# rflamino/monte_carlo_retirement

Hardware: AMD Instinct MI355X
Metric: paths/sec (whole node), config.json scenario, 833-month paths, success-count only (higher is better)
Workload: dtype f64

## Files before the change

### monte_carlo_retirement_amd/csrc/mcr_hip.hip

```cpp

#include <hip/hip_runtime.h>

#include <climits>
#include <cmath>
#include <cstdarg>
#include <cstdio>
#include <cstdlib>
#include <cstring>
#include <algorithm>
#include <mutex>
#include <thread>
#include <type_traits>
#include <utility>
#include <vector>

#include "mcr_device.h"
#include "mcr_numpy_rng.h"
#include "mcr_screen.h"
#include "mcr_host.h"

namespace mcr {

constexpr int kMaxSegments = 8;
constexpr int kRngHistorySchemes = 3;
// ... 1001 lines not shown
    if (kSliced && seg >= 0 && seg < io.seg_q - 1) {
        const bool hand_over = seg == 0 || __hip_atomic_load(&seg_ok_s, __ATOMIC_RELAXED, __HIP_MEMORY_SCOPE_WORKGROUP) != 0;
        if (hand_over) {
            *seg_at(0) = b1; *seg_at(1) = b2; *seg_at(2) = c1; *seg_at(3) = c2;
            if (ANNUAL) { *seg_at(4) = gacc1; *seg_at(5) = gacc2; }
            *seg_at(6) = infl;
            store_bits(seg_at(7), (alive ? 1ull : 0ull) | (succeeded ? 2ull : 0ull) | ((unsigned long long)(ruin_bin + 1) << 8) | ((unsigned long long)done_years << 24));
            store_bits(seg_at(8), ((unsigned long long)carry.w3 << 32) | (unsigned long long)carry.w2);
            for (int k = 0; k < P.n_lock_slots; ++k) *seg_at(kSegFixedFields + k) = lock_lds[(size_t)k * kBlock + tid];
            if (MODE >= 1) {
                *seg_at(9) = start_balance; *seg_at(10) = infl_ret;
                *seg_at(11) = sum_col[0]; *seg_at(12) = sum_col[kBlock]; *seg_at(13) = sum_col[2 * kBlock];
            }
            __builtin_amdgcn_fence(__ATOMIC_RELEASE, "agent");
        }
        __syncthreads();
        if (threadIdx.x == 0)
            __hip_atomic_store(io.seg_flags + (size_t)seg_block * (size_t)io.seg_q + (size_t)seg, hand_over ? 1u : 2u, __ATOMIC_RELEASE, __HIP_MEMORY_SCOPE_AGENT);
        return;
    }

    if (P.total_months % kMPY != 0) {
        if (succeeded) {
            const bool tf = annual_gain_taxes<false, TANY, ANNUAL, T1, T2, MM, TOL, EQR>(P, L, b1, c1, b2, c2, gacc1, gacc2);
            if (tf) {
                succeeded = false; ruin_bin = ry + 1;
                if (kSumLds) sum_col[2 * kBlock] = (double)ry; else ytr_bits = f64_bits((double)ry);
                if constexpr (OUT) RM.month = kMPY * ry;
            }
            if constexpr (kBins) YB.last = b1 + b2;
            else put_sample(P.trajectory_len - 1, b1 + b2, infl);
        }
        if constexpr (kBins) year_bins_row(io.yb, YB.L, YB.k++, valid, P.trajectory_len - 1, true, YB.last, infl, -1, kNanBits);
    }
    const double final_balance = fmax(0.0, b1 + b2);

    if (kSumLds) { fy_gross = sum_col[0]; fy_real = sum_col[kBlock]; ytr_bits = f64_bits(sum_col[2 * kBlock]); }
    if (kSummary && valid) {
        const mcr_outputs& o = io.out;
        if (o.start_balance) o.start_balance[li] = start_balance;
        if (o.final_balance) o.final_balance[li] = final_balance;
        if (o.years_to_ruin) store_bits(&o.years_to_ruin[li], ytr_bits);
        if (o.first_year_gross_withdrawal) o.first_year_gross_withdrawal[li] = fy_gross;
        if (o.first_year_real_gross_withdrawal) o.first_year_real_gross_withdrawal[li] = fy_real;
        if (o.inflation_at_retirement) o.inflation_at_retirement[li] = infl_ret;
        if (o.success) o.success[li] = succeeded ? 1 : 0;
    }
#ifdef MCR_K1_TIMELINE
    if (MODE == 0 && RNG == 0 && io.path_seeds && (threadIdx.x & 63) == 0) {
        unsigned long long* tl = (unsigned long long*)io.path_seeds + ((size_t)blockIdx.x * 4 + (threadIdx.x >> 6)) * 3;
        tl[0] = tl_t0; tl[1] = wall_clock64();
        tl[2] = ((unsigned long long)__builtin_amdgcn_s_getreg(20 | (31 << 11)) << 32) | __builtin_amdgcn_s_getreg(4 | (31 << 11));
    }
#endif
    const unsigned long long ok = __builtin_amdgcn_ballot_w64(valid && succeeded);
    if (kFan) {
        if ((threadIdx.x & 63) == 0) blk[fan_j] = (unsigned int)__popcll(ok);
        if constexpr (kScnFan) {
            const int fan_n = late_arg<int32_t>(offsetof(KernelIO, fan_n));
            const uint64_t n_paths = late_arg<uint64_t>(offsetof(KernelIO, n_paths));
            uint64_t* const fan_ctr = late_arg<uint64_t*>(offsetof(KernelIO, out) + offsetof(mcr_outputs, counters));
            uint64_t* const fan_masks = late_arg<uint64_t*>(offsetof(KernelIO, fan_masks));
            if (fan_masks && (threadIdx.x & 63) == 0) fan_masks[(size_t)fan_j * ((n_paths + 63) >> 6) + path_block] = ok;
            if constexpr (OUT) {
                double* const fan_final = late_arg<double*>(offsetof(KernelIO, fan_rows) + offsetof(KernelIO::FanRows, final_balance));
                double* const fan_ruin = late_arg<double*>(offsetof(KernelIO, fan_rows) + offsetof(KernelIO::FanRows, years_to_ruin));
                const int64_t row_stride = late_arg<int64_t>(offsetof(KernelIO, fan_rows) + offsetof(KernelIO::FanRows, row_stride));
                const uint64_t col = (uint64_t)path_block * kPaths + (threadIdx.x & 63);
                if (col < n_paths) {
                    const size_t at = (size_t)fan_j * (size_t)row_stride + (size_t)col;
                    if (fan_final) store_bits(&fan_final[at], succeeded ? f64_bits(final_balance) : kNanBits);
                    if (fan_ruin) store_bits(&fan_ruin[at], RM.month < 0 ? kNanBits : f64_bits((double)RM.month / (double)kMPY));
                }
            }
            __syncthreads();
            if (threadIdx.x < (unsigned)fan_n && fan_ctr) {
                uint64_t* c = fan_ctr + (size_t)threadIdx.x * MCR_N_COUNTERS;
                const uint64_t first = (uint64_t)path_block * kPaths;
                const uint64_t cnt = n_paths - first < (uint64_t)kPaths ? n_paths - first : (uint64_t)kPaths;
                atomicAdd((unsigned long long*)&c[MCR_CTR_SUCCESS], (unsigned long long)blk[threadIdx.x]);
                atomicAdd((unsigned long long*)&c[MCR_CTR_PATHS], (unsigned long long)cnt);
            }
            return;
        }
        __syncthreads();
        uint64_t* const fan_ctr = kGrid ? cell->counters : io.out.counters;
        if (threadIdx.x < (unsigned)io.fan_n && fan_ctr) {
            uint64_t* c = fan_ctr + (size_t)threadIdx.x * MCR_N_COUNTERS;
            const uint64_t first = (uint64_t)path_block * kPaths;
            const uint64_t cnt = io.n_paths - first < (uint64_t)kPaths ? io.n_paths - first : (uint64_t)kPaths;
            atomicAdd((unsigned long long*)&c[MCR_CTR_SUCCESS], (unsigned long long)blk[threadIdx.x]);
            atomicAdd((unsigned long long*)&c[MCR_CTR_PATHS], (unsigned long long)cnt);
        }
        return;
    }
    if ((threadIdx.x & 63) == 0) atomicAdd(&blk[0], (unsigned int)__popcll(ok));
    const bool want_bins = io.out.ruin_year_bins != nullptr || io.out.wr_obs_counts != nullptr;
    if (want_bins && valid) {
        if (ruin_bin >= 0) atomicAdd(&blk[1 + ruin_bin], 1u);
        atomicAdd(&blk[1 + (ry + 2) + done_years], 1u);
    }
    if ((PHASE == 0 || PHASE == 3) && n_hist > 0 && valid && succeeded) {
        const double* __restrict__ e = io.out.hist_edges;
        if (final_balance >= e[0] && final_balance <= e[n_hist]) {
            int lo = 0, hi = n_hist;
            while (hi - lo > 1) {
                const int mid = (lo + hi) >> 1;
                if (e[mid] <= final_balance) lo = mid; else hi = mid;
            }
            atomicAdd(&blk[n_blk + lo], 1u);
        }
    }
    if constexpr (kBins) { if (io.yb.final_success && valid && succeeded) atomicAdd(&YB.L.fin[year_bins_cell(YB.L.edges, YB.L.n, final_balance)], 1u); }
    __syncthreads();
    if constexpr (kBins) year_bins_flush_final(io.yb, YB.L);
    uint64_t* ctr = io.out.counters ? io.out.counters + (kCand ? (size_t)io.cand_out[cand] * MCR_N_COUNTERS : 0) : nullptr;
    if (threadIdx.x == 0 && ctr) {
        atomicAdd((unsigned long long*)&ctr[MCR_CTR_SUCCESS], (unsigned long long)blk[0]);
        const uint64_t first = (uint64_t)path_block * kPaths;
        const uint64_t cnt = io.n_paths - first < (uint64_t)kPaths ? io.n_paths - first : (uint64_t)kPaths;
        if constexpr (LIST) {
            const uint64_t list_n = *io.path_list_count;
            atomicAdd((unsigned long long*)&ctr[MCR_CTR_PATHS], (unsigned long long)(list_n - first < (uint64_t)kPaths ? list_n - first : (uint64_t)kPaths));
        } else
        atomicAdd((unsigned long long*)&ctr[MCR_CTR_PATHS], (unsigned long long)cnt);
    }
    if (want_bins) {
        for (int k = threadIdx.x; k < ry + 2; k += kPaths) {
            if (io.out.ruin_year_bins && blk[1 + k])
                atomicAdd((unsigned long long*)&io.out.ruin_year_bins[k], (unsigned long long)blk[1 + k]);
        }
        for (int y = threadIdx.x; y < ry; y += kPaths) {
            unsigned int c = 0;
            for (int d = y + 1; d <= ry; ++d) c += blk[1 + (ry + 2) + d];
            if (io.out.wr_obs_counts && c)
                atomicAdd((unsigned long long*)&io.out.wr_obs_counts[y], (unsigned long long)c);
        }
    }
    for (int k = threadIdx.x; k < n_hist; k += kPaths)
        if (blk[n_blk + k]) atomicAdd((unsigned long long*)&io.out.hist_bins[k], (unsigned long long)blk[n_blk + k]);
}

struct ScreenIO {
    uint64_t seed, path_begin, n_paths;
    uint32_t stream_id, reserved;
    uint64_t* counters;
    uint64_t* wr_obs_counts;
    uint32_t* list;
    uint32_t* list_count;
    uint8_t* cls;
    float* min_ratio;
    float* final_total;
};
template <int TAXED, bool EQR, bool HOOK = false>
__global__ __launch_bounds__(kBlock, 8) void screen_kernel(const ScreenParams S, const ScreenIO io) {
    static_assert(TAXED >= 0 && TAXED <= 3 && (!EQR || TAXED == 3), "TAXED is path_kernel's mask; equal rates need both assets taxed");
    constexpr bool T1 = (TAXED & 1) != 0, T2 = (TAXED & 2) != 0;
    __shared__ unsigned int safe_s;
    if (threadIdx.x == 0) safe_s = 0u;
    __syncthreads();
    const uint64_t local = (uint64_t)blockIdx.x * kBlock + threadIdx.x;
    const bool valid = local < io.n_paths;
    const uint64_t path = io.path_begin + (valid ? local : io.n_paths - 1);
    const PhiloxPath PQ = philox_path(path, io.stream_id, io.seed);
    float b1 = S.b1_0, b2 = S.b2_0, c1 = b1, c2 = b2, infl = 1.0f;
    float peak = b1 + b2;
    float contrib = S.contrib, k1 = contrib * S.alloc1, k2 = contrib - k1;
    bool ok = __builtin_fminf(b1, b2) > kScreenMinBalance;
    [[maybe_unused]] float min_ratio = __builtin_inff();
    PairCarry carry{0u, 0u};
    const int wm = S.working_months, total = S.total_months;
    int moy = 0;
    const int prio_t1 = (total / 2) & ~1, prio_t2 = ((total * 3) / 4) & ~1, prio_t3 = ((total * 9) / 10) & ~1;
    int prio_next = prio_t1;
    __builtin_amdgcn_s_setprio(3);
    for (int row = 0; row < total; row += 2) {
        if (__builtin_amdgcn_ballot_w64(ok) == 0ull) break;
        if (row == prio_next) {
            if (row == prio_t1) __builtin_amdgcn_s_setprio(2);
            else if (row == prio_t2) __builtin_amdgcn_s_setprio(1);
            else if (row == prio_t3) __builtin_amdgcn_s_setprio(0);
            prio_next = prio_from(prio_t1, prio_t2, prio_t3, row + 2);
        }
        float g[6];
        if (PQ.hi_uniform) {
            if ((row & 2) == 0) screen_factors2<0, true>(S, PQ, io.seed, (uint32_t)row >> 2, carry, g);
            else screen_factors2<1, true>(S, PQ, io.seed, (uint32_t)row >> 2, carry, g);
        } else {
            if ((row & 2) == 0) screen_factors2<0, false>(S, PQ, io.seed, (uint32_t)row >> 2, carry, g);
            else screen_factors2<1, false>(S, PQ, io.seed, (uint32_t)row >> 2, carry, g);
        }
#pragma unroll
        for (int r = 0; r < 2; ++r) {
            const int m = row + r;
            if (m >= total) break;
            const float g1 = g[3 * r], ginf = g[3 * r + 1], g2 = g[3 * r + 2];
            if (m < wm) {
                if (moy == kMPY) {
                    moy = 0;
                    if (S.contrib_grows) { contrib *= S.contrib_growth_factor; k1 = contrib * S.alloc1; k2 = contrib - k1; }
                }
                ++moy;
                b1 *= g1; b2 *= g2; infl *= ginf;
                b1 += k1; c1 += k1; b2 += k2; c2 += k2;
            } else {
                const float price = infl;
                float income = S.expenses * price;
                if ((unsigned)(m - S.s0) < S.n0) income = __builtin_fmaf(-S.sa0, price, income);
                if ((unsigned)(m - S.s1) < S.n1) income = __builtin_fmaf(-S.sa1, price, income);
                const float need = __builtin_fmaxf(0.0f, income);
                b1 *= g1; b2 *= g2; infl *= ginf;
                const float v1 = T1 ? __builtin_fmaf(-__builtin_fmaxf(0.0f, b1 - c1), S.rate1, b1) : b1;
                const float v2 = T2 ? __builtin_fmaf(-__builtin_fmaxf(0.0f, b2 - c2), EQR ? S.rate1 : S.rate2, b2) : b2;
                const float cap = v1 + v2;
                ok = ok && cap >= kScreenNeedMargin * need && cap >= peak * (1.0f / kScreenPeakDiv);
                const float inv_cap = __builtin_amdgcn_rcpf(cap);
                const float phi = __builtin_fminf(need, cap) * inv_cap;
                if constexpr (HOOK) { if (need > 0.0f) min_ratio = __builtin_fminf(min_ratio, cap * __builtin_amdgcn_rcpf(need)); }
                b1 = __builtin_fmaf(-b1, phi, b1); c1 = __builtin_fmaf(-c1, phi, c1);
                b2 = __builtin_fmaf(-b2, phi, b2); c2 = __builtin_fmaf(-c2, phi, c2);
            }
            peak = __builtin_fmaxf(peak, screen_rebalance<TAXED, EQR>(S, b1, c1, b2, c2));
            ok = ok && __builtin_fminf(b1, b2) > kScreenMinBalance;
        }
    }
    ok = ok && peak < kScreenMaxTotal;
    const bool safe = valid && ok, doubt = valid && !ok;
    const unsigned long long safe_mask = __builtin_amdgcn_ballot_w64(safe), doubt_mask = __builtin_amdgcn_ballot_w64(doubt);
    const unsigned int lane = threadIdx.x & 63u;
    if (lane == 0u && safe_mask) atomicAdd(&safe_s, (unsigned int)__popcll(safe_mask));
    if (io.list && doubt_mask) {
        unsigned int base = 0u;
        if (lane == 0u) base = atomicAdd(io.list_count, (unsigned int)__popcll(doubt_mask));
        base = (unsigned int)__builtin_amdgcn_readfirstlane((int)base);
        const unsigned int before = __builtin_amdgcn_mbcnt_hi((unsigned int)(doubt_mask >> 32), __builtin_amdgcn_mbcnt_lo((unsigned int)doubt_mask, 0u));
        if (doubt) io.list[base + before] = (uint32_t)local;
    }
    if constexpr (HOOK) {
        if (valid) {
            if (io.cls) io.cls[local] = ok ? MCR_SCREEN_SAFE : MCR_SCREEN_DOUBTFUL;
            if (io.min_ratio) io.min_ratio[local] = min_ratio;
            if (io.final_total) io.final_total[local] = b1 + b2;
        }
    }
    __syncthreads();
    const unsigned int n_safe = safe_s;
    if (n_safe == 0u) return;
    if (threadIdx.x == 0 && io.counters) {
        atomicAdd((unsigned long long*)&io.counters[MCR_CTR_SUCCESS], (unsigned long long)n_safe);
        atomicAdd((unsigned long long*)&io.counters[MCR_CTR_PATHS], (unsigned long long)n_safe);
    }
    if (io.wr_obs_counts)
        for (int y = threadIdx.x; y < S.retirement_years; y += kBlock) atomicAdd((unsigned long long*)&io.wr_obs_counts[y], (unsigned long long)n_safe);
}

__global__ void exp_forms_kernel(const double* in, double* out, int64_t n) {
    __shared__ double tab[kTabDoubles], tab_c[kTabDoubles];
    load_math_tables(tab, threadIdx.x, blockDim.x);
    load_math_tables<true>(tab_c, threadIdx.x, blockDim.x);
    __syncthreads();
    const int64_t i = (int64_t)blockIdx.x * blockDim.x + threadIdx.x;
    if (i >= n) return;
    out[2 * i] = fexp<true>(in[i], tab, MathRegs::literals_path());
    out[2 * i + 1] = fexp<true, true>(in[i], tab_c, MathRegs::literals_path());
}
__global__ void helper_kernel(int which, const DevParams P, const double* in, double* out, int64_t n) {
    __shared__ double tab[kTabDoubles];
    load_math_tables(tab, threadIdx.x, blockDim.x);
    __syncthreads();
    const int64_t i = (int64_t)blockIdx.x * blockDim.x + threadIdx.x;
    if (i >= n) return;
    switch (which) {
        case MCR_HELPER_WITHDRAW: {
            const double* x = in + 5 * i;
            double bal = x[0], cb = x[1], g, nt;
            const double rate = (x[3] != 0.0 && x[4] > 0.0) ? x[4] : 0.0;
            withdraw(bal, cb, x[2], rate, g, nt);
            out[4 * i + 0] = bal; out[4 * i + 1] = cb; out[4 * i + 2] = g; out[4 * i + 3] = nt;
            break;
        }
        case MCR_HELPER_NLV: {
            const double* x = in + 4 * i;
            const double rate = (x[2] != 0.0 && x[3] > 0.0) ? x[3] : 0.0;
            out[i] = net_liquidation_value(x[0], x[1], rate);
            break;
        }
        case MCR_HELPER_REBALANCE: {
            const double* x = in + 4 * i;
            double b1 = x[0], c1 = x[1], b2 = x[2], c2 = x[3];
            rebalance(lane_params(P), b1, c1, b2, c2);
            out[4 * i + 0] = b1; out[4 * i + 1] = c1; out[4 * i + 2] = b2; out[4 * i + 3] = c2;
            break;
        }
        case MCR_HELPER_ANNUAL_TAX: {
            const double* x = in + 6 * i;
            double b1 = x[0], c1 = x[1], b2 = x[2], c2 = x[3];
            const bool tf = annual_gain_taxes(P, lane_params(P), b1, c1, b2, c2, x[4], x[5]);
            out[5 * i + 0] = b1; out[5 * i + 1] = c1; out[5 * i + 2] = b2; out[5 * i + 3] = c2;
            out[5 * i + 4] = tf ? 1.0 : 0.0;
            break;
        }
        case MCR_HELPER_MONTHLY_GROSS: {
            const double* x = in + 3 * i;
            out[i] = monthly_gross(x[0] / (double)kMPY, x[1] / sqrt((double)kMPY), x[2], tab);
            break;
        }
        case MCR_HELPER_MATH_EXP: out[i] = fexp(in[i], tab, MathRegs::literals()); break;
        case MCR_HELPER_MATH_DIV: out[i] = fdiv(in[2 * i], in[2 * i + 1]); break;
        case MCR_HELPER_MATH_DIV_PATH: out[i] = fdiv<false>(in[2 * i], in[2 * i + 1]); break;
        case MCR_HELPER_MATH_SQRT: out[i] = fsqrt(in[i]); break;
        case MCR_HELPER_WITHDRAW2_PATH: {
            const double* x = in + 6 * i;
            const LaneParams L = lane_params(P);
            double b1 = x[0], c1 = x[1], b2 = x[3], c2 = x[4], g1, n1, g2, n2;
            switch (P.tax_mask) {
                case 0: withdraw2<false, false>(b1, c1, x[2], L.real_rate1, g1, n1, b2, c2, x[5], L.real_rate2, g2, n2); break;
                case 1: withdraw2<true, false>(b1, c1, x[2], L.real_rate1, g1, n1, b2, c2, x[5], L.real_rate2, g2, n2); break;
                case 2: withdraw2<false, true>(b1, c1, x[2], L.real_rate1, g1, n1, b2, c2, x[5], L.real_rate2, g2, n2); break;
                default: withdraw2<true, true>(b1, c1, x[2], L.real_rate1, g1, n1, b2, c2, x[5], L.real_rate2, g2, n2); break;
            }
            double* o = out + 8 * i;
            o[0] = b1; o[1] = c1; o[2] = g1; o[3] = n1; o[4] = b2; o[5] = c2; o[6] = g2; o[7] = n2;
            break;
        }
        case MCR_HELPER_NLV2_PATH: {
            const double* x = in + 4 * i;
            const LaneParams L = lane_params(P);
            double v1, v2;
            switch (P.tax_mask) {
                case 0: net_liquidation_values2<false, false>(x[0], x[1], L.real_rate1, x[2], x[3], L.real_rate2, v1, v2); break;
                case 1: net_liquidation_values2<true, false>(x[0], x[1], L.real_rate1, x[2], x[3], L.real_rate2, v1, v2); break;
                case 2: net_liquidation_values2<false, true>(x[0], x[1], L.real_rate1, x[2], x[3], L.real_rate2, v1, v2); break;
                default: net_liquidation_values2<true, true>(x[0], x[1], L.real_rate1, x[2], x[3], L.real_rate2, v1, v2); break;
            }
            out[2 * i] = v1; out[2 * i + 1] = v2;
            break;
        }
        case MCR_HELPER_REBALANCE_PATH: {
            const double* x = in + 4 * i;
            double b1 = x[0], c1 = x[1], b2 = x[2], c2 = x[3];
            if (P.any_real_rate) rebalance_path<true>(lane_params(P), b1, c1, b2, c2);
            else rebalance_path<false>(lane_params(P), b1, c1, b2, c2);
            out[4 * i + 0] = b1; out[4 * i + 1] = c1; out[4 * i + 2] = b2; out[4 * i + 3] = c2;
            break;
        }
        case MCR_HELPER_ANNUAL_TAX_PATH: {
            const double* x = in + 6 * i;
            double b1 = x[0], c1 = x[1], b2 = x[2], c2 = x[3];
            const LaneParams L = lane_params(P);
            bool tf;
#define MCR_ATAX(T1_, T2_) (P.any_annual_tax ? annual_gain_taxes<false, (T1_) || (T2_), true, T1_, T2_>(P, L, b1, c1, b2, c2, x[4], x[5]) \
                                             : annual_gain_taxes<false, (T1_) || (T2_), false, T1_, T2_>(P, L, b1, c1, b2, c2, x[4], x[5]))
            switch (P.tax_mask) {
                case 0: tf = MCR_ATAX(false, false); break;
                case 1: tf = MCR_ATAX(true, false); break;
                case 2: tf = MCR_ATAX(false, true); break;
                default: tf = MCR_ATAX(true, true); break;
            }
#undef MCR_ATAX
            out[5 * i + 0] = b1; out[5 * i + 1] = c1; out[5 * i + 2] = b2; out[5 * i + 3] = c2;
            out[5 * i + 4] = tf ? 1.0 : 0.0;
            break;
        }
        case MCR_HELPER_WITHDRAW_MONTH: {
            const double* x = in + 5 * i;
            double b1 = x[0], c1 = x[1], b2 = x[2], c2 = x[3];
            const double need = x[4];
            double gross, net;
            if (P.exact_month) {
                const LaneParams L = lane_params(P);
                double cap1, cap2, g1, n1, g2, n2;
                net_liquidation_values2<true, true>(b1, c1, L.real_rate1, b2, c2, L.real_rate2, cap1, cap2);
                const double cap = cap1 + cap2, target = fmin(need, cap);
                double prop1 = fdiv<false>(cap1, cap);
                if (!(cap > kEps)) prop1 = P.alloc1;
                withdraw2<true, true>(b1, c1, target * prop1, L.real_rate1, g1, n1, b2, c2, target * (1.0 - prop1), L.real_rate2, g2, n2);
                gross = g1 + g2; net = n1 + n2;
            } else {
// ... 686 lines not shown
    fill_io_rng(io, rng, device_path_seeds);
    io.stream_id = stream_id; io.path_begin = path_begin; io.n_paths = n_paths;
    return io;
}
static mcr_outputs counters_only(uint64_t* counters) {
    mcr_outputs o;
    std::memset(&o, 0, sizeof(o));
    o.counters = counters;
    return o;
}

template <int V> using int_c = std::integral_constant<int, V>;
template <typename F> static inline void for_bool(bool b, F&& f) { if (b) f(std::true_type{}); else f(std::false_type{}); }
template <typename F> static inline void for_tax_variant(const DevParams& d, F&& f) {
    for_bool(d.any_annual_tax, [&](auto A) {
        switch (d.tax_mask) { case 0: f(int_c<0>{}, A); break; case 1: f(int_c<1>{}, A); break; case 2: f(int_c<2>{}, A); break; default: f(int_c<3>{}, A); break; }
    });
}
template <typename F> static inline void for_growth_form(int gf, F&& f) {
    if (gf == (kGrowthNarrowExp | kGrowthRhoZero)) f(int_c<kGrowthNarrowExp | kGrowthRhoZero>{});
    else if (gf == kGrowthNarrowExp) f(int_c<kGrowthNarrowExp>{});
    else f(int_c<0>{});
}
template <int T, typename F> static inline void for_month_form(int mf, F&& f) {
    if constexpr (T == 3 && !kExactMonthDefault) { if (mf == kMonthEqualRates) { f(int_c<kMonthEqualRates>{}); return; } }
    f(int_c<0>{});
}
template <typename F> static inline void for_stream_form(int sf, F&& f) {
    if constexpr (!kExactMonthDefault) { if (sf == kStreamsInRegs) { f(int_c<kStreamsInRegs>{}); return; } }
    f(int_c<0>{});
}
template <int MODE, int RNG, bool ANNUAL, bool XS> constexpr bool kHasGrowthForms = MODE == 0 && RNG == 0 && !ANNUAL && !XS;
template <typename F> static inline void for_output_mode(int mode, F&& f) {
    if (mode == 2) f(int_c<2>{}); else if (mode == 1) f(int_c<1>{}); else f(int_c<0>{});
}

template <typename F> static inline void for_whole_path_variant(const DevParams& d, uint32_t rng_kind, bool xs, bool exact, F&& f) {
    auto with_stream = [&](auto R) {
        if (xs) {
            if (exact) f(R, int_c<3>{}, std::true_type{}, std::true_type{}, std::true_type{});
            else f(R, int_c<3>{}, std::true_type{}, std::true_type{}, std::false_type{});
        } else if constexpr (decltype(R)::value == 0) {
            for_tax_variant(d, [&](auto T, auto A) { f(R, T, A, std::false_type{}, std::false_type{}); });
        } else {
            for_bool(d.any_annual_tax, [&](auto A) {
                if (d.any_real_rate) f(R, int_c<3>{}, A, std::false_type{}, std::false_type{});
                else f(R, int_c<0>{}, A, std::false_type{}, std::false_type{});
            });
        }
    };
    if (rng_kind == (uint32_t)kRngHistorySchemes) with_stream(int_c<kRngHistorySchemes>{});
    else if (rng_kind == MCR_RNG_HISTORY) with_stream(int_c<(int)MCR_RNG_HISTORY>{});
    else if (rng_kind == MCR_RNG_NUMPY) with_stream(int_c<(int)MCR_RNG_NUMPY>{});
    else with_stream(int_c<0>{});
}
static bool needs_exact_month(const DevParams& d) { return d.exact_month && !kExactMonthDefault; }
static bool needs_generic_variant(const DevParams& d) { return d.n_extra_streams > 0 || needs_exact_month(d); }
static int check_barrier_counts(const DevParams& d, int producers = 1) {
    if (d.total_months == d.working_months + kMPY * d.retirement_years && (producers == 1 || d.total_months >= 1)) return MCR_OK;
    set_error("internal: total_months != working_months + 12 retirement_years");
    return MCR_ERR_INVALID_ARG;
}

struct StreamAlloc {
    void* p = nullptr;
    hipStream_t stream;
    explicit StreamAlloc(hipStream_t s) : stream(s) {}
    StreamAlloc(const StreamAlloc&) = delete;
    StreamAlloc& operator=(const StreamAlloc&) = delete;
    ~StreamAlloc() { (void)release(); }
    bool alloc(size_t bytes) {
        if (hipMallocAsync(&p, bytes, stream) == hipSuccess) return true;
        (void)hipGetLastError();
        p = nullptr;
        return false;
    }
    hipError_t release() {
        if (!p) return hipSuccess;
        const hipError_t e = hipFreeAsync(p, stream);
        p = nullptr;
        return e;
    }
};
struct SegmentHandOver {
    StreamAlloc mem;
    explicit SegmentHandOver(hipStream_t s) : mem(s) {}
    bool attach(KernelIO& io, const SegmentPlan& plan, int n_fields, hipError_t* zeroed) {
        const size_t state_bytes = (size_t)plan.n_split * (size_t)n_fields * kBlock * sizeof(double);
        const size_t flag_bytes = (size_t)plan.n_split * (size_t)plan.q * sizeof(unsigned int);
        if (!mem.alloc(state_bytes + flag_bytes)) return false;
        *zeroed = hipMemsetAsync((char*)mem.p + state_bytes, 0, flag_bytes, mem.stream);
        if (*zeroed != hipSuccess) return true;
        io.seg_state = (double*)mem.p;
        io.seg_flags = (unsigned int*)((char*)mem.p + state_bytes);
        io.seg_n_split = plan.n_split; io.seg_n_full = plan.n_full; io.seg_q = plan.q; io.seg_max_polls = plan.max_polls;
        for (int k = 0; k <= plan.q; ++k) io.seg_year[k] = plan.year[k];
        return true;
    }
    hipError_t release() { return mem.release(); }
};

static bool screen_qualified(const DevParams& d) {
    return !kExactMonthDefault && !d.any_annual_tax && !d.exact_month && d.n_extra_streams == 0 && stream_form_qualified(d) == kStreamsInRegs;
}
constexpr uint64_t kScreenMinPathsDefault = 500000;
static const char* const kClassicKnobs[] = {"MCR_K1_SEGMENTS", "MCR_K1_SEGMENTS_ALWAYS", "MCR_K1_SEGMENT_ORDER", "MCR_K1_SEGMENT_POLLS",
                                            "MCR_K1_GROWTH_FORM", "MCR_K1_MONTH_FORM", "MCR_K1_STREAM_FORM"};
constexpr int kRerunProducersDefault = 1;
constexpr double kRerunTwoProducersMaxList = 80000.0;
static int rerun_producers_of(int* producers, double expected_list = -1.0) {
    *producers = (expected_list >= 0.0 && expected_list <= kRerunTwoProducersMaxList) ? 2 : kRerunProducersDefault;
    if (const char* e = std::getenv("MCR_K1_RERUN_PRODUCERS"); e && *e) {
        if ((e[0] != '1' && e[0] != '2') || e[1] != '\0') { set_error("MCR_K1_RERUN_PRODUCERS=%s: 1 (the 256-path form) or 2 (64 paths, two producer waves)", e); return MCR_ERR_INVALID_ARG; }
        *producers = e[0] - '0';
    }
    return MCR_OK;
}
static int screen_route_of(const DevParams& d, const mcr_rng* rng, uint64_t n_paths, int hist_n_bins, bool* screened) {
    *screened = false;
    int force = -1;
    if (const char* e = std::getenv("MCR_K1_SCREEN"); e && *e) {
        if ((e[0] != '0' && e[0] != '1') || e[1] != '\0') { set_error("MCR_K1_SCREEN=%s: 0 (never) or 1 (whenever the launch qualifies)", e); return MCR_ERR_INVALID_ARG; }
        force = e[0] - '0';
    }
    int producers = 0;
    if (int rc = rerun_producers_of(&producers)) return rc;
    if (force == 0 || !screen_qualified(d) || (rng && rng->kind != MCR_RNG_PHILOX) || hist_n_bins != 0) return MCR_OK;
    if (n_paths == 0 || n_paths > (uint64_t)UINT32_MAX) return MCR_OK;
    for (const char* knob : kClassicKnobs) { const char* e = std::getenv(knob); if (e && *e) return MCR_OK; }
    uint64_t min_paths = kScreenMinPathsDefault;
    if (const char* e = std::getenv("MCR_K1_SCREEN_MIN_PATHS"); e && *e) {
        char* end = nullptr;
        min_paths = std::strtoull(e, &end, 10);
        if (*end != '\0') { set_error("MCR_K1_SCREEN_MIN_PATHS=%s: a path count", e); return MCR_ERR_INVALID_ARG; }
    }
    *screened = force == 1 || n_paths >= min_paths;
    return MCR_OK;
}
static double screen_expected() {
    const char* e = std::getenv("MCR_K1_SCREEN_EXPECTED");
    const double v = (e && *e) ? std::strtod(e, nullptr) : 0.08;
    return v > 0.0 ? v : 0.08;
}
static ScreenParams screen_params(const DevParams& d) {
    const double log2e = 1.4426950408889634074;
    ScreenParams s;
    std::memset(&s, 0, sizeof(s));
    s.a1 = (float)(d.a1 * log2e); s.b1 = (float)(d.b1 * log2e);
    s.ainf = (float)(d.ainf * log2e); s.binf_rho = (float)(d.binf_rho * log2e); s.binf_rho_c = (float)(d.binf_rho_c * log2e);
    s.aprem = (float)(d.aprem * log2e); s.bprem = (float)(d.bprem * log2e);
    const double b1 = d.initial_balance * d.alloc1;
    s.b1_0 = (float)b1; s.b2_0 = (float)(d.initial_balance - b1);
    s.contrib = (float)d.monthly_contribution; s.contrib_growth_factor = (float)d.contrib_growth_factor;
    s.expenses = (float)d.monthly_expenses; s.alloc1 = (float)d.alloc1;
    s.rate1 = (float)d.real_rate1; s.rate2 = (float)d.real_rate2;
    s.ar1 = (float)(d.alloc1 * d.real_rate1); s.ar2 = (float)(d.alloc2 * d.real_rate2);
    const int wm = d.working_months;
    auto to_row = [&](int32_t m) { return m > INT32_MAX - wm ? INT32_MAX : m + wm; };
    auto window_months = [](int first, int end) { return end > first ? (uint32_t)(end - first) : 0u; };
    if (d.n_streams > 0) { s.sa0 = (float)d.streams[0].amount_keep; s.s0 = to_row(d.streams[0].start_month); s.n0 = window_months(s.s0, to_row(d.streams[0].end_month)); }
    if (d.n_streams > 1) { s.sa1 = (float)d.streams[1].amount_keep; s.s1 = to_row(d.streams[1].start_month); s.n1 = window_months(s.s1, to_row(d.streams[1].end_month)); }
    s.working_months = wm; s.retirement_years = d.retirement_years; s.total_months = d.total_months; s.contrib_grows = d.contrib_grows;
    return s;
}
template <bool HOOK>
static void launch_screen_kernel(const DevParams& d, const ScreenParams& sp, const ScreenIO& sio, dim3 grid, hipStream_t stream) {
    const bool eqr = month_form_qualified(d) == kMonthEqualRates;
    switch (d.tax_mask) {
        case 0: hipLaunchKernelGGL((screen_kernel<0, false, HOOK>), grid, dim3(kBlock), 0, stream, sp, sio); break;
        case 1: hipLaunchKernelGGL((screen_kernel<1, false, HOOK>), grid, dim3(kBlock), 0, stream, sp, sio); break;
        case 2: hipLaunchKernelGGL((screen_kernel<2, false, HOOK>), grid, dim3(kBlock), 0, stream, sp, sio); break;
        default:
            if (eqr) hipLaunchKernelGGL((screen_kernel<3, true, HOOK>), grid, dim3(kBlock), 0, stream, sp, sio);
            else hipLaunchKernelGGL((screen_kernel<3, false, HOOK>), grid, dim3(kBlock), 0, stream, sp, sio);
    }
}
static int launch_screened(DevParams d, KernelIO io, hipStream_t stream) {
    const uint64_t n = io.n_paths;
    int producers = 1;
    int rc = rerun_producers_of(&producers, (double)n * screen_expected());
    if (rc != MCR_OK) return rc;
    StreamAlloc mem(stream);
    if (!mem.alloc(4 * (size_t)n + 8)) return MCR_ERR_UNSUPPORTED;
    uint32_t* const count = (uint32_t*)mem.p;
    uint32_t* const list = (uint32_t*)((char*)mem.p + 8);
    hipError_t e = hipMemsetAsync(count, 0, 8, stream);
    if (e != hipSuccess) return hip_fail(e, "screened launch: zeroing the list's count");
    const dim3 grid((unsigned)((n + kBlock - 1) / kBlock)), block(kBlock);
    ScreenIO sio;
    std::memset(&sio, 0, sizeof(sio));
    sio.seed = io.seed; sio.path_begin = io.path_begin; sio.n_paths = n; sio.stream_id = io.stream_id;
    sio.counters = io.out.counters; sio.wr_obs_counts = io.out.wr_obs_counts; sio.list = list; sio.list_count = count;
    launch_screen_kernel<false>(d, screen_params(d), sio, grid, stream);
    e = hipGetLastError();
    if (e != hipSuccess) return hip_fail(e, "screen_kernel launch");
    bool split = (double)n * screen_expected() / 64.0 <= (double)split_max_waves();
    rc = split ? check_barrier_counts(d, producers) : MCR_OK;
    if (rc != MCR_OK) return rc;
    size_t lds = 0;
    rc = plan_path_kernel_lds(d, 0, MCR_RNG_PHILOX, false, split, 0, &lds);
    if (rc != MCR_OK) return rc;
    io.path_list = list; io.path_list_count = count;
    const DevParams* const no_cand = nullptr;
    const int mf = month_form_qualified(d);
    if (split && producers == 2) {
        const dim3 grid64((unsigned)((n + 63) / 64));
        for_tax_variant(d, [&](auto T, auto A) {
            if constexpr (!decltype(A)::value && !kExactMonthDefault)
                for_month_form<decltype(T)::value>(mf, [&](auto F) {
                    hipLaunchKernelGGL((path_kernel<0, 0, decltype(T)::value, false, false, 0, true, false, false, 0, decltype(F)::value, kStreamsInRegs, false, true, 2>),
                                       grid64, dim3(3 * 64), lds, stream, d, io, no_cand);
                });
        });
    } else if (split) {
        for_tax_variant(d, [&](auto T, auto A) {
            if constexpr (!decltype(A)::value && !kExactMonthDefault)
                for_month_form<decltype(T)::value>(mf, [&](auto F) {
                    hipLaunchKernelGGL((path_kernel<0, 0, decltype(T)::value, false, false, 0, true, false, false, 0, decltype(F)::value, kStreamsInRegs, false, true>),
                                       grid, dim3(2 * kBlock), lds, stream, d, io, no_cand);
                });
        });
    } else {
        const int gf = growth_form_qualified(d);
        for_tax_variant(d, [&](auto T, auto A) {
            if constexpr (!decltype(A)::value && !kExactMonthDefault)
                for_growth_form(gf, [&](auto G) {
                    for_month_form<decltype(T)::value>(mf, [&](auto F) {
                        hipLaunchKernelGGL((path_kernel<0, 0, decltype(T)::value, false, false, 0, false, false, false, decltype(G)::value, decltype(F)::value, kStreamsInRegs, false, true>),
                                           grid, block, lds, stream, d, io, no_cand);
                    });
                });
        });
    }
    e = hipGetLastError();
    const hipError_t ef = mem.release();
    if (e != hipSuccess) return hip_fail(e, "path_kernel launch (screened re-run)");
    if (ef != hipSuccess) return hip_fail(ef, "screened launch: list release");
    return MCR_OK;
}

static int launch_paths(const mcr_params* p, const mcr_rng* rng, uint32_t stream_id, uint64_t path_begin,
                        uint64_t n_paths, int32_t wm, const double* injected, const mcr_outputs* out,
                        hipStream_t stream) {
    DevParams d;
    std::vector<DevStream> extra;
    int rc = derive_params(p, wm, &d, &extra);
    if (rc != MCR_OK) return rc;
    rc = check_rng(rng);
    if (rc != MCR_OK) return rc;
    if (!out) { set_error("null outputs"); return MCR_ERR_INVALID_ARG; }
    if (n_paths == 0) return MCR_OK;
    if (n_paths > (uint64_t)INT32_MAX * kBlock) { set_error("n_paths too large for one launch"); return MCR_ERR_INVALID_ARG; }
    if (path_begin + n_paths < path_begin) { set_error("path range overflows 64 bits"); return MCR_ERR_INVALID_ARG; }
    const bool want_traj = out->trajectory || out->real_trajectory || out->withdrawal_rate_trajectory;
    const bool want_summary = out->start_balance || out->final_balance || out->years_to_ruin ||
                              out->first_year_gross_withdrawal || out->first_year_real_gross_withdrawal ||
                              out->inflation_at_retirement || out->success;
    KernelIO io = make_io(rng, rng->path_seeds, stream_id, path_begin, n_paths);
    io.injected = injected; io.out = *out;
    if (io.out.path_stride <= 0) io.out.path_stride = (int64_t)n_paths;
    if (want_traj && (uint64_t)io.out.path_stride < n_paths) {
        set_error("path_stride %lld < n_paths %llu", (long long)io.out.path_stride, (unsigned long long)n_paths);
        return MCR_ERR_INVALID_ARG;
    }
    const uint32_t rng_kind = rng->kind;
    const bool np_rng = rng_kind != MCR_RNG_PHILOX;
    if (io.out.hist_bins == nullptr || io.out.hist_n_bins == 0) { io.out.hist_bins = nullptr; io.out.hist_edges = nullptr; io.out.hist_n_bins = 0; }
    if (io.out.hist_bins && (io.out.hist_n_bins < 0 || io.out.hist_n_bins > MCR_MAX_HIST_BINS || !io.out.hist_edges)) {
        set_error("hist_bins requested with hist_n_bins = %d (1..%d) / hist_edges = %p", io.out.hist_n_bins, MCR_MAX_HIST_BINS, (const void*)io.out.hist_edges);
        return MCR_ERR_INVALID_ARG;
    }
    const dim3 grid((unsigned)((n_paths + kBlock - 1) / kBlock)), block(kBlock);
    const int mode = injected ? 2 : (want_traj ? 2 : (want_summary ? 1 : 0));
    bool split = !injected && !np_rng && mode == 0 && (uint64_t)grid.x * (kBlock / 64) <= split_max_waves();
    if (split && (rc = check_barrier_counts(d)) != MCR_OK) return rc;
    size_t lds = 0;
    rc = plan_path_kernel_lds(d, mode, rng_kind, injected != nullptr, split, io.out.hist_n_bins, &lds, 0, rng->history_months);
    if (rc != MCR_OK) return rc;
    if (split && (d.n_lock_slots < d.n_lock_slots_total || needs_generic_variant(d))) {
        split = false;
        rc = plan_path_kernel_lds(d, mode, rng_kind, false, false, io.out.hist_n_bins, &lds);
        if (rc != MCR_OK) return rc;
    }
    const bool exact = needs_exact_month(d);
    const bool xs = d.n_lock_slots < d.n_lock_slots_total || needs_generic_variant(d);
    const char* seg_order = segment_order_env();
    if (seg_order && (np_rng || injected || xs || split)) {
        set_error("MCR_K1_SEGMENT_ORDER=%s set on a launch that is not time-sliced (%s)", seg_order,
                  rng_kind == MCR_RNG_HISTORY ? "history stream" : np_rng ? "NumPy stream" : injected ? "injected shocks" : xs ? "extended streams / exact month" : "producer / consumer split");
        return MCR_ERR_INVALID_ARG;
    }
    int gf = 0;
    rc = growth_form_of(d, !np_rng && !injected && !xs && !split && mode == 0 && !d.any_annual_tax, &gf);
    if (rc != MCR_OK) return rc;
    int mf = 0;
    rc = month_form_of(d, !np_rng && !injected && !xs && !split && mode == 0 && !d.any_annual_tax, &mf);
    if (rc != MCR_OK) return rc;
    int sf = 0;
    rc = stream_form_of(d, !np_rng && !injected && !xs && !split && mode == 0 && !d.any_annual_tax, &sf);
    if (rc != MCR_OK) return rc;
    if (!injected && !np_rng && mode == 0 && !xs) {
        bool screened = false;
        rc = screen_route_of(d, rng, n_paths, io.out.hist_n_bins, &screened);
        if (rc != MCR_OK) return rc;
        if (screened) {
            rc = launch_screened(d, io, stream);
            if (rc != MCR_ERR_UNSUPPORTED) return rc;
        }
    }
    StreamSideBlock side;
    rc = side.attach(d, extra, grid.x, stream);
    if (rc != MCR_OK) { (void)side.release(stream); return rc; }
    const DevParams* const no_cand = nullptr;
    auto launch_whole_path = [&]() {
        for_output_mode(mode, [&](auto M) {
            for_whole_path_variant(d, kernel_rng_kind(rng), xs, exact, [&](auto R, auto T, auto A, auto X, auto EX) {
                if constexpr (kHasGrowthForms<decltype(M)::value, decltype(R)::value, decltype(A)::value, decltype(X)::value>) {
                    for_growth_form(gf, [&](auto G) {
                        for_month_form<decltype(T)::value>(mf, [&](auto F) {
                            for_stream_form(sf, [&](auto S) {
                                hipLaunchKernelGGL((path_kernel<0, 0, decltype(T)::value, false, false, 0, false, false, kExactMonthDefault, decltype(G)::value, decltype(F)::value, decltype(S)::value>),
                                                   grid, block, lds, stream, d, io, no_cand);
                            });
                        });
                    });
                } else {
                    hipLaunchKernelGGL((path_kernel<decltype(M)::value, decltype(R)::value, decltype(T)::value, decltype(A)::value, false, 0, false,
                                                    decltype(X)::value, (decltype(X)::value && decltype(EX)::value) || kExactMonthDefault>),
// ... 2145 lines not shown
```

### monte_carlo_retirement_amd/csrc/mcr_screen.h

```cpp
#pragma once

#include "mcr_device.h"

namespace mcr {

constexpr float kScreenNeedMargin = 24.0f;
constexpr float kScreenPeakDiv = 64.0f;
constexpr float kScreenMinBalance = 1.0f;
constexpr float kScreenMaxTotal = 1e30f;

struct ScreenParams {
    float a1, b1, ainf, binf_rho, binf_rho_c, aprem, bprem;
    float b1_0, b2_0;
    float contrib, contrib_growth_factor, expenses, alloc1;
    float rate1, rate2, ar1, ar2;
    float sa0, sa1;
    int32_t s0, s1;
    uint32_t n0, n1;
    int32_t working_months, retirement_years, total_months, contrib_grows;
};

template <int HALF, bool UNIFORM>
__device__ __forceinline__ void screen_factors2(const ScreenParams& S, const PhiloxPath& Q, uint64_t seed, uint32_t t, PairCarry& C, float (&g)[6]) {
    float rad[3], trig[6];
    auto parts = [&](uint32_t xr, uint32_t xa, int i) {
        const float u = __builtin_fmaf((float)xr, 0x1p-32f, 0x1p-33f);
        rad[i] = __builtin_amdgcn_sqrtf(-1.3862943611198906f * __builtin_amdgcn_logf(u));
        const float rev = (float)xa * 0x1p-32f;
        trig[2 * i] = __builtin_amdgcn_cosf(rev);
        trig[2 * i + 1] = __builtin_amdgcn_sinf(rev);
    };
    uint32_t x[4];
    if (HALF == 0) {
        philox_path_rounds<UNIFORM>(Q, 3u * t, (uint32_t)seed, (uint32_t)(seed >> 32), x);
        parts(x[0], x[1], 0);
        parts(x[2], x[3], 1);
        philox_path_rounds<UNIFORM>(Q, 3u * t + 1u, (uint32_t)seed, (uint32_t)(seed >> 32), x);
        parts(x[0], x[1], 2);
        C.w2 = x[2]; C.w3 = x[3];
    } else {
        parts(C.w2, C.w3, 0);
        philox_path_rounds<UNIFORM>(Q, 3u * t + 2u, (uint32_t)seed, (uint32_t)(seed >> 32), x);
        parts(x[0], x[1], 1);
        parts(x[2], x[3], 2);
    }
#pragma unroll
    for (int r = 0; r < 2; ++r) {
        const int je = 3 * r, ji = 3 * r + 1, jp = 3 * r + 2;
        const float ne = rad[je >> 1] * trig[je], ni = rad[ji >> 1] * trig[ji], np = rad[jp >> 1] * trig[jp];
        const float g1 = __builtin_amdgcn_exp2f(__builtin_fmaf(S.b1, ne, S.a1));
        const float ginf = __builtin_amdgcn_exp2f(__builtin_fmaf(S.binf_rho, ne, __builtin_fmaf(S.binf_rho_c, ni, S.ainf)));
        const float gprem = __builtin_amdgcn_exp2f(__builtin_fmaf(S.bprem, np, S.aprem));
        g[3 * r + 0] = g1; g[3 * r + 1] = ginf; g[3 * r + 2] = ginf * gprem;
    }
}

template <int TAXED, bool EQR>
__device__ __forceinline__ float screen_rebalance(const ScreenParams& S, float& b1, float& c1, float& b2, float& c2) {
    const float total = b1 + b2;
    const float drift1 = __builtin_fmaf(-total, S.alloc1, b1);
    const bool sell1 = drift1 > 0.0f;
    const float bs = sell1 ? b1 : b2, cs = sell1 ? c1 : c2;
    const float drift = __builtin_fabsf(drift1);
    float fraction_sold, net_purchase;
    if (TAXED != 0) {
        const float rate_s = EQR ? S.rate1 : sell1 ? S.rate1 : S.rate2;
        const float ar_s = sell1 ? S.ar1 : S.ar2;
        const float G = __builtin_fmaxf(0.0f, bs - cs);
        fraction_sold = __builtin_fminf(1.0f, drift * __builtin_amdgcn_rcpf(__builtin_fmaf(-ar_s, G, bs)));
        net_purchase = fraction_sold * __builtin_fmaf(-G, rate_s, bs);
    } else {
        fraction_sold = __builtin_fminf(1.0f, drift * __builtin_amdgcn_rcpf(bs));
        net_purchase = fraction_sold * bs;
    }
    const float nbs = __builtin_fmaf(-bs, fraction_sold, bs), ncs = __builtin_fmaf(-cs, fraction_sold, cs);
    const float r1b = b1 + net_purchase, r1c = c1 + net_purchase, r2b = b2 + net_purchase, r2c = c2 + net_purchase;
    b1 = sell1 ? nbs : r1b; c1 = sell1 ? ncs : r1c;
    b2 = sell1 ? r2b : nbs; c2 = sell1 ? r2c : ncs;
    return total;
}

}
```

Baseline: 380.9 million.

## Streamline screen kernel inner loop with log-space inflation and precomputed expense levels

Restructures the float screening kernel's per-month math. Inflation is tracked as a log2 level, with one exp2 at withdrawal, and the premium factor is fused into a single exp2. Expense levels for the four income-stream window combinations are precomputed on the host and picked with selects. A compile-time RHO0 variant drops the correlation FMA, min-balance checks are folded into a running minimum, the wave ballot early-exit runs only every 16 rows, constants are pinned in VGPRs, and two fminf clamps are removed. Together these cut ALU and transcendental work per month. The risks are screen classification drifting when the removed clamps or the delayed exit matter, and extra template instantiations.

```diff
diff --git a/monte_carlo_retirement_amd/csrc/mcr_hip.hip b/monte_carlo_retirement_amd/csrc/mcr_hip.hip
--- a/monte_carlo_retirement_amd/csrc/mcr_hip.hip
+++ b/monte_carlo_retirement_amd/csrc/mcr_hip.hip
@@ -1177,7 +1177,7 @@
     float* min_ratio;
     float* final_total;
 };
-template <int TAXED, bool EQR, bool HOOK = false>
+template <int TAXED, bool EQR, bool RHO0, bool HOOK = false>
 __global__ __launch_bounds__(kBlock, 8) void screen_kernel(const ScreenParams S, const ScreenIO io) {
     static_assert(TAXED >= 0 && TAXED <= 3 && (!EQR || TAXED == 3), "TAXED is path_kernel's mask; equal rates need both assets taxed");
     constexpr bool T1 = (TAXED & 1) != 0, T2 = (TAXED & 2) != 0;
@@ -1188,19 +1188,23 @@
     const bool valid = local < io.n_paths;
     const uint64_t path = io.path_begin + (valid ? local : io.n_paths - 1);
     const PhiloxPath PQ = philox_path(path, io.stream_id, io.seed);
-    float b1 = S.b1_0, b2 = S.b2_0, c1 = b1, c2 = b2, infl = 1.0f;
+    float b1 = S.b1_0, b2 = S.b2_0, c1 = b1, c2 = b2;
+    float lvl = 0.0f;
     float peak = b1 + b2;
     float contrib = S.contrib, k1 = contrib * S.alloc1, k2 = contrib - k1;
-    bool ok = __builtin_fminf(b1, b2) > kScreenMinBalance;
+    bool ok = true;
+    float rmin = __builtin_fminf(b1, b2);
     [[maybe_unused]] float min_ratio = __builtin_inff();
     PairCarry carry{0u, 0u};
+    ScreenConsts K{S.a1, S.ainf, S.aprem, S.ar1, S.ar2};
+    asm volatile("" : "+v"(K.a1), "+v"(K.ainf), "+v"(K.aprem), "+v"(K.ar1), "+v"(K.ar2));
     const int wm = S.working_months, total = S.total_months;
     int moy = 0;
     const int prio_t1 = (total / 2) & ~1, prio_t2 = ((total * 3) / 4) & ~1, prio_t3 = ((total * 9) / 10) & ~1;
     int prio_next = prio_t1;
     __builtin_amdgcn_s_setprio(3);
     for (int row = 0; row < total; row += 2) {
-        if (__builtin_amdgcn_ballot_w64(ok) == 0ull) break;
+        if ((row & 14) == 0 && __builtin_amdgcn_ballot_w64(ok && rmin > kScreenMinBalance) == 0ull) break;
         if (row == prio_next) {
             if (row == prio_t1) __builtin_amdgcn_s_setprio(2);
             else if (row == prio_t2) __builtin_amdgcn_s_setprio(1);
@@ -1209,46 +1213,51 @@
         }
         float g[6];
         if (PQ.hi_uniform) {
-            if ((row & 2) == 0) screen_factors2<0, true>(S, PQ, io.seed, (uint32_t)row >> 2, carry, g);
-            else screen_factors2<1, true>(S, PQ, io.seed, (uint32_t)row >> 2, carry, g);
+            if ((row & 2) == 0) screen_factors2<0, true, RHO0>(S, K, PQ, io.seed, (uint32_t)row >> 2, carry, g);
+            else screen_factors2<1, true, RHO0>(S, K, PQ, io.seed, (uint32_t)row >> 2, carry, g);
         } else {
-            if ((row & 2) == 0) screen_factors2<0, false>(S, PQ, io.seed, (uint32_t)row >> 2, carry, g);
-            else screen_factors2<1, false>(S, PQ, io.seed, (uint32_t)row >> 2, carry, g);
+            if ((row & 2) == 0) screen_factors2<0, false, RHO0>(S, K, PQ, io.seed, (uint32_t)row >> 2, carry, g);
+            else screen_factors2<1, false, RHO0>(S, K, PQ, io.seed, (uint32_t)row >> 2, carry, g);
         }
 #pragma unroll
         for (int r = 0; r < 2; ++r) {
             const int m = row + r;
             if (m >= total) break;
-            const float g1 = g[3 * r], ginf = g[3 * r + 1], g2 = g[3 * r + 2];
+            const float g1 = g[3 * r], xinf = g[3 * r + 1], g2 = g[3 * r + 2];
             if (m < wm) {
                 if (moy == kMPY) {
                     moy = 0;
-                    if (S.contrib_grows) { contrib *= S.contrib_growth_factor; k1 = contrib * S.alloc1; k2 = contrib - k1; }
+                    if (S.contrib_grows) {
+                        asm volatile("");
+                        contrib *= S.contrib_growth_factor; k1 = contrib * S.alloc1; k2 = contrib - k1;
+                    }
                 }
                 ++moy;
-                b1 *= g1; b2 *= g2; infl *= ginf;
+                b1 *= g1; b2 *= g2; lvl += xinf;
                 b1 += k1; c1 += k1; b2 += k2; c2 += k2;
             } else {
-                const float price = infl;
-                float income = S.expenses * price;
-                if ((unsigned)(m - S.s0) < S.n0) income = __builtin_fmaf(-S.sa0, price, income);
-                if ((unsigned)(m - S.s1) < S.n1) income = __builtin_fmaf(-S.sa1, price, income);
-                const float need = __builtin_fmaxf(0.0f, income);
-                b1 *= g1; b2 *= g2; infl *= ginf;
+                const float price = __builtin_amdgcn_exp2f(lvl);
+                const bool w0 = (unsigned)(m - S.s0) < S.n0, w1 = (unsigned)(m - S.s1) < S.n1;
+                const uint32_t on0 = w1 ? __builtin_bit_cast(uint32_t, S.e11) : __builtin_bit_cast(uint32_t, S.e10);
+                const uint32_t off0 = w1 ? __builtin_bit_cast(uint32_t, S.e01) : __builtin_bit_cast(uint32_t, S.e00);
+                const float level = __builtin_bit_cast(float, w0 ? on0 : off0);
+                const float need = __builtin_fmaxf(0.0f, price * level);
+                b1 *= g1; b2 *= g2; lvl += xinf;
                 const float v1 = T1 ? __builtin_fmaf(-__builtin_fmaxf(0.0f, b1 - c1), S.rate1, b1) : b1;
                 const float v2 = T2 ? __builtin_fmaf(-__builtin_fmaxf(0.0f, b2 - c2), EQR ? S.rate1 : S.rate2, b2) : b2;
                 const float cap = v1 + v2;
                 ok = ok && cap >= kScreenNeedMargin * need && cap >= peak * (1.0f / kScreenPeakDiv);
                 const float inv_cap = __builtin_amdgcn_rcpf(cap);
-                const float phi = __builtin_fminf(need, cap) * inv_cap;
+                const float phi = need * inv_cap;
                 if constexpr (HOOK) { if (need > 0.0f) min_ratio = __builtin_fminf(min_ratio, cap * __builtin_amdgcn_rcpf(need)); }
                 b1 = __builtin_fmaf(-b1, phi, b1); c1 = __builtin_fmaf(-c1, phi, c1);
                 b2 = __builtin_fmaf(-b2, phi, b2); c2 = __builtin_fmaf(-c2, phi, c2);
             }
-            peak = __builtin_fmaxf(peak, screen_rebalance<TAXED, EQR>(S, b1, c1, b2, c2));
-            ok = ok && __builtin_fminf(b1, b2) > kScreenMinBalance;
-        }
-    }
+            peak = __builtin_fmaxf(peak, screen_rebalance<TAXED, EQR>(S, K, b1, c1, b2, c2));
+            rmin = __builtin_fminf(rmin, __builtin_fminf(b1, b2));
+        }
+    }
+    ok = ok && rmin > kScreenMinBalance;
     ok = ok && peak < kScreenMaxTotal;
     const bool safe = valid && ok, doubt = valid && !ok;
     const unsigned long long safe_mask = __builtin_amdgcn_ballot_w64(safe), doubt_mask = __builtin_amdgcn_ballot_w64(doubt);
@@ -2241,28 +2250,36 @@
     const double b1 = d.initial_balance * d.alloc1;
     s.b1_0 = (float)b1; s.b2_0 = (float)(d.initial_balance - b1);
     s.contrib = (float)d.monthly_contribution; s.contrib_growth_factor = (float)d.contrib_growth_factor;
-    s.expenses = (float)d.monthly_expenses; s.alloc1 = (float)d.alloc1;
+    s.alloc1 = (float)d.alloc1;
+    const double keep0 = d.n_streams > 0 ? d.streams[0].amount_keep : 0.0, keep1 = d.n_streams > 1 ? d.streams[1].amount_keep : 0.0;
+    s.e00 = (float)d.monthly_expenses; s.e10 = (float)(d.monthly_expenses - keep0);
+    s.e01 = (float)(d.monthly_expenses - keep1); s.e11 = (float)(d.monthly_expenses - keep0 - keep1);
     s.rate1 = (float)d.real_rate1; s.rate2 = (float)d.real_rate2;
     s.ar1 = (float)(d.alloc1 * d.real_rate1); s.ar2 = (float)(d.alloc2 * d.real_rate2);
     const int wm = d.working_months;
     auto to_row = [&](int32_t m) { return m > INT32_MAX - wm ? INT32_MAX : m + wm; };
     auto window_months = [](int first, int end) { return end > first ? (uint32_t)(end - first) : 0u; };
-    if (d.n_streams > 0) { s.sa0 = (float)d.streams[0].amount_keep; s.s0 = to_row(d.streams[0].start_month); s.n0 = window_months(s.s0, to_row(d.streams[0].end_month)); }
-    if (d.n_streams > 1) { s.sa1 = (float)d.streams[1].amount_keep; s.s1 = to_row(d.streams[1].start_month); s.n1 = window_months(s.s1, to_row(d.streams[1].end_month)); }
+    if (d.n_streams > 0) { s.s0 = to_row(d.streams[0].start_month); s.n0 = window_months(s.s0, to_row(d.streams[0].end_month)); }
+    if (d.n_streams > 1) { s.s1 = to_row(d.streams[1].start_month); s.n1 = window_months(s.s1, to_row(d.streams[1].end_month)); }
     s.working_months = wm; s.retirement_years = d.retirement_years; s.total_months = d.total_months; s.contrib_grows = d.contrib_grows;
     return s;
 }
 template <bool HOOK>
 static void launch_screen_kernel(const DevParams& d, const ScreenParams& sp, const ScreenIO& sio, dim3 grid, hipStream_t stream) {
     const bool eqr = month_form_qualified(d) == kMonthEqualRates;
-    switch (d.tax_mask) {
-        case 0: hipLaunchKernelGGL((screen_kernel<0, false, HOOK>), grid, dim3(kBlock), 0, stream, sp, sio); break;
-        case 1: hipLaunchKernelGGL((screen_kernel<1, false, HOOK>), grid, dim3(kBlock), 0, stream, sp, sio); break;
-        case 2: hipLaunchKernelGGL((screen_kernel<2, false, HOOK>), grid, dim3(kBlock), 0, stream, sp, sio); break;
-        default:
-            if (eqr) hipLaunchKernelGGL((screen_kernel<3, true, HOOK>), grid, dim3(kBlock), 0, stream, sp, sio);
-            else hipLaunchKernelGGL((screen_kernel<3, false, HOOK>), grid, dim3(kBlock), 0, stream, sp, sio);
-    }
+    const bool rho0 = d.rho == 0.0;
+    auto go = [&](auto R) {
+        constexpr bool RHO0 = decltype(R)::value;
+        switch (d.tax_mask) {
+            case 0: hipLaunchKernelGGL((screen_kernel<0, false, RHO0, HOOK>), grid, dim3(kBlock), 0, stream, sp, sio); break;
+            case 1: hipLaunchKernelGGL((screen_kernel<1, false, RHO0, HOOK>), grid, dim3(kBlock), 0, stream, sp, sio); break;
+            case 2: hipLaunchKernelGGL((screen_kernel<2, false, RHO0, HOOK>), grid, dim3(kBlock), 0, stream, sp, sio); break;
+            default:
+                if (eqr) hipLaunchKernelGGL((screen_kernel<3, true, RHO0, HOOK>), grid, dim3(kBlock), 0, stream, sp, sio);
+                else hipLaunchKernelGGL((screen_kernel<3, false, RHO0, HOOK>), grid, dim3(kBlock), 0, stream, sp, sio);
+        }
+    };
+    if (rho0) go(std::true_type{}); else go(std::false_type{});
 }
 static int launch_screened(DevParams d, KernelIO io, hipStream_t stream) {
     const uint64_t n = io.n_paths;
diff --git a/monte_carlo_retirement_amd/csrc/mcr_screen.h b/monte_carlo_retirement_amd/csrc/mcr_screen.h
--- a/monte_carlo_retirement_amd/csrc/mcr_screen.h
+++ b/monte_carlo_retirement_amd/csrc/mcr_screen.h
@@ -12,16 +12,18 @@
 struct ScreenParams {
     float a1, b1, ainf, binf_rho, binf_rho_c, aprem, bprem;
     float b1_0, b2_0;
-    float contrib, contrib_growth_factor, expenses, alloc1;
+    float contrib, contrib_growth_factor, alloc1;
     float rate1, rate2, ar1, ar2;
-    float sa0, sa1;
+    float e00, e10, e01, e11;
     int32_t s0, s1;
     uint32_t n0, n1;
     int32_t working_months, retirement_years, total_months, contrib_grows;
 };
 
-template <int HALF, bool UNIFORM>
-__device__ __forceinline__ void screen_factors2(const ScreenParams& S, const PhiloxPath& Q, uint64_t seed, uint32_t t, PairCarry& C, float (&g)[6]) {
+struct ScreenConsts { float a1, ainf, aprem, ar1, ar2; };
+
+template <int HALF, bool UNIFORM, bool RHO0>
+__device__ __forceinline__ void screen_factors2(const ScreenParams& S, const ScreenConsts& K, const PhiloxPath& Q, uint64_t seed, uint32_t t, PairCarry& C, float (&g)[6]) {
     float rad[3], trig[6];
     auto parts = [&](uint32_t xr, uint32_t xa, int i) {
         const float u = __builtin_fmaf((float)xr, 0x1p-32f, 0x1p-33f);
@@ -48,15 +50,16 @@
     for (int r = 0; r < 2; ++r) {
         const int je = 3 * r, ji = 3 * r + 1, jp = 3 * r + 2;
         const float ne = rad[je >> 1] * trig[je], ni = rad[ji >> 1] * trig[ji], np = rad[jp >> 1] * trig[jp];
-        const float g1 = __builtin_amdgcn_exp2f(__builtin_fmaf(S.b1, ne, S.a1));
-        const float ginf = __builtin_amdgcn_exp2f(__builtin_fmaf(S.binf_rho, ne, __builtin_fmaf(S.binf_rho_c, ni, S.ainf)));
-        const float gprem = __builtin_amdgcn_exp2f(__builtin_fmaf(S.bprem, np, S.aprem));
-        g[3 * r + 0] = g1; g[3 * r + 1] = ginf; g[3 * r + 2] = ginf * gprem;
+        const float g1 = __builtin_amdgcn_exp2f(__builtin_fmaf(S.b1, ne, K.a1));
+        float xinf = __builtin_fmaf(S.binf_rho_c, ni, K.ainf);
+        if (!RHO0) xinf = __builtin_fmaf(S.binf_rho, ne, xinf);
+        const float xprem = __builtin_fmaf(S.bprem, np, K.aprem);
+        g[3 * r + 0] = g1; g[3 * r + 1] = xinf; g[3 * r + 2] = __builtin_amdgcn_exp2f(xinf + xprem);
     }
 }
 
 template <int TAXED, bool EQR>
-__device__ __forceinline__ float screen_rebalance(const ScreenParams& S, float& b1, float& c1, float& b2, float& c2) {
+__device__ __forceinline__ float screen_rebalance(const ScreenParams& S, const ScreenConsts& K, float& b1, float& c1, float& b2, float& c2) {
     const float total = b1 + b2;
     const float drift1 = __builtin_fmaf(-total, S.alloc1, b1);
     const bool sell1 = drift1 > 0.0f;
@@ -65,12 +68,12 @@
     float fraction_sold, net_purchase;
     if (TAXED != 0) {
         const float rate_s = EQR ? S.rate1 : sell1 ? S.rate1 : S.rate2;
-        const float ar_s = sell1 ? S.ar1 : S.ar2;
+        const float ar_s = sell1 ? K.ar1 : K.ar2;
         const float G = __builtin_fmaxf(0.0f, bs - cs);
-        fraction_sold = __builtin_fminf(1.0f, drift * __builtin_amdgcn_rcpf(__builtin_fmaf(-ar_s, G, bs)));
+        fraction_sold = drift * __builtin_amdgcn_rcpf(__builtin_fmaf(-ar_s, G, bs));
         net_purchase = fraction_sold * __builtin_fmaf(-G, rate_s, bs);
     } else {
-        fraction_sold = __builtin_fminf(1.0f, drift * __builtin_amdgcn_rcpf(bs));
+        fraction_sold = drift * __builtin_amdgcn_rcpf(bs);
         net_purchase = fraction_sold * bs;
     }
     const float nbs = __builtin_fmaf(-bs, fraction_sold, bs), ncs = __builtin_fmaf(-cs, fraction_sold, cs);
```

Measured after the change: 422.7 million (median of 6 runs). +11.0%, better.
